# Sewer56/dxt-lossless-transform

Hardware: AMD Instinct MI355X
Metric: GiB/s BC blocks transformed (fwd+inv) (higher is better)
Workload: dtype u8

## Files before the change

dxt-lossless-transform_amd/csrc/batch_api.cpp:

```cpp
#include <hip/hip_runtime_api.h>

#include <algorithm>
#include <cstring>
#include <vector>

#include "../../include/dxtlt_gfx950.h"
#include "batch_tables.h"
#include "bcn_launch.h"
#include "granule_launch.h"
#include "host_common.h"

namespace {

using namespace dxtlt_host;
using dxtlt::BatchEntry;

const char* const kDeviceFormatText = "batch item: format must be 1..5 (BC1..BC5), 6 (BC6H) or 7 (BC7; 6 and 7 are this build's own formats; "
                                      "pixel formats 8 and 9 go through dxtlt_transform_batch_host or the calls of dxtlt_pixels.h)";
const char* const kHostFormatText = "batch item: format must be 1..5 (BC1..BC5), 6 (BC6H), 7 (BC7), 8 (4-byte pixels) or 9 (3-byte pixels; "
                                    "6 to 9 are this build's own formats)";

inline bool pixel_item_overlaps(const DxtltBatchItem& it)
{
    if (!is_pixel_format(it.format) || it.len == 0)
        return false;
    const uintptr_t a = reinterpret_cast<uintptr_t>(it.d_input), b = reinterpret_cast<uintptr_t>(it.d_output);
    return a < b + it.len && b < a + it.len;
}

int32_t launch_pixel_item(const DxtltBatchItem& it, void* stream)
{
    const uint64_t pixels = it.len / item_block_bytes(it.format);
    return pixel_device_range(pixel_bytes_of(it.format), it.inverse != 0, it.d_input, it.d_output, pixels, 0, pixels,
                              pixel_decorrelate_of(it.decorrelation_mode),
                              pixel_layout_of(it.split_alpha_endpoints != 0, it.split_colour_endpoints != 0), stream);
}

thread_local dxtlt_host::TableRing g_ring;

const bool kTableByCopyEngine = dxtlt::experiment_env("DXTLT_BATCH_TABLE_COPY") != nullptr && dxtlt::experiment_env("DXTLT_BATCH_TABLE_COPY")[0] == '1';

}

dxtlt_host::TableRing& dxtlt_host::thread_table_ring() { return g_ring; }

hipError_t dxtlt_host::upload_table(TableSlot* slot, size_t bytes, hipStream_t stream)
{
    if (kTableByCopyEngine)
        return hipMemcpyAsync(slot->dev, slot->host, bytes, hipMemcpyHostToDevice, stream);
    return dxtlt::launch_table_upload(slot->host_mapped, slot->dev, bytes, stream);
}

void dxtlt_host::release_batch_thread_tables() { g_ring.release(); }

int32_t dxtlt_host::batch_item_defect(const DxtltBatchItem& it, int max_format, bool host_call)
{
    if (it.format < 1 || it.format > max_format)
        return fail(kInvalidArgument, host_call ? kHostFormatText : kDeviceFormatText);
    if (it.len % item_block_bytes(it.format) != 0)
        return fail(kInvalidLength, "batch item: len is not a multiple of the block size");
    if (it.decorrelation_mode > 3 && dxtlt::format_has_colour(it.format))
        return fail(kInvalidArgument, "batch item: decorrelation_mode must be 0..3");
    if (it.len > 0 && (it.d_input == nullptr || it.d_output == nullptr))
        return fail(kInvalidArgument, host_call ? "batch item: NULL buffer with len > 0" : "batch item: NULL device buffer with len > 0");
    if (pixel_item_overlaps(it))
        return fail(kInvalidArgument, "batch item: pixel input and output overlap");
    if (host_call && it.len >= (size_t(4) << 30))
        return fail(kInvalidArgument, "batch item of 4 GiB or more: use the single-buffer entry point");
    return kOk;
}

namespace {

inline dxtlt::Settings item_settings(const DxtltBatchItem& it)
{
    dxtlt::Settings s{};
    s.variant = it.decorrelation_mode;
    s.split_alpha = it.split_alpha_endpoints != 0;
    s.split_colour = it.split_colour_endpoints != 0;
    return dxtlt::effective_settings((dxtlt::Format)it.format, s);
}

struct TileLaunch {
    int key = 0;
    std::vector<BatchEntry> entries;
    uint32_t wgs = 0;
    uint32_t uniform_wgs = 0;
    bool strided = false;
    int64_t src_stride = 0, dst_stride = 0;
    bool wide = false;
    size_t at = 0, entry_bytes = 0;

    dxtlt::Format format() const { return (dxtlt::Format)((key >> 5) + 1); }
    bool inverse() const { return ((key >> 4) & 1) != 0; }
};

using GranuleEntry = dxtlt::granule::BatchEntry;
struct GranuleLaunch {
    std::vector<GranuleEntry> entries, tails;
    std::vector<uint32_t> coarse;
    uint64_t wgs = 0;
    size_t items = 0;
    size_t at = 0, entry_bytes = 0, tail_bytes = 0, bytes = 0;
};

struct BatchPlan {
    GranuleLaunch granules[4];
    std::vector<TileLaunch> tiles;
    std::vector<size_t> singles;
    std::vector<size_t> pixels;
    size_t table_bytes = 0;
};
inline int granule_format(int q) { return q < 2 ? 7 : 6; }

int32_t plan_batch(const DxtltBatchItem* items, size_t count, bool pixels_allowed, BatchPlan& plan)
{
    if (count == 0)
        return kOk;
    if (items == nullptr)
        return fail(kInvalidArgument, "NULL item array with count > 0");
    for (size_t i = 0; i < count; ++i)
        if (int32_t rc = batch_item_defect(items[i], pixels_allowed ? 9 : 7, false); rc != kOk)
            return rc;
    for (const int format : {7, 6}) {
        uint64_t granules[2] = {0, 0};
        for (size_t i = 0; i < count; ++i)
            if (items[i].format == format)
                granules[items[i].inverse ? 1 : 0] += items[i].len / 16 / 1024;
        if (granules[0] > 0xFFFFFFull || granules[1] > 0xFFFFFFull)
            return fail(kInvalidArgument, dxtlt::granule::named(format, "batch too large for one launch (256 GiB or more of ", " in one direction)"));
    }

    int launch_of_key[5 * 2 * 16];
    for (int& l : launch_of_key)
        l = -1;
    for (size_t i = 0; i < count; ++i) {
        const DxtltBatchItem& it = items[i];
        if (it.len == 0 || dxtlt::granule::is_granule_format(it.format))
            continue;
        if (is_pixel_format(it.format)) {
            plan.pixels.push_back(i);
            continue;
        }
        if (it.len >= (size_t(64) << 30))
            return fail(kInvalidArgument, "batch item of 64 GiB or more: use the single-buffer entry point");
        const dxtlt::Settings s = item_settings(it);
        const int key = (((it.format - 1) * 2 + (it.inverse ? 1 : 0)) << 4) | settings_code(s);
        int li = launch_of_key[key];
        BatchEntry e{};
        e.src = static_cast<const uint8_t*>(it.d_input);
        e.dst = static_cast<uint8_t*>(it.d_output);
        e.blocks = it.len / item_block_bytes(it.format);
        e.first_wg = li >= 0 ? plan.tiles[(size_t)li].wgs : 0;
        const uint32_t wgs = dxtlt::plan_batch_entry((dxtlt::Format)it.format, it.inverse != 0, s, e);
        if (wgs == 0xFFFFFFFFu) {
            plan.singles.push_back(i);
            continue;
        }
        if (li < 0) {
            li = launch_of_key[key] = (int)plan.tiles.size();
            plan.tiles.emplace_back();
            plan.tiles.back().key = key;
            plan.tiles.back().uniform_wgs = wgs;
        }
        TileLaunch& l = plan.tiles[(size_t)li];
        if ((uint64_t)l.wgs + wgs > 0xFFFFFFull)
            return fail(kInvalidArgument, "batch too large for one launch (64 GiB or more of one format, direction and settings)");
        l.wgs += wgs;
        l.entries.push_back(e);
        if (wgs != l.uniform_wgs)
            l.uniform_wgs = 0;
    }
    std::sort(plan.tiles.begin(), plan.tiles.end(), [](const TileLaunch& a, const TileLaunch& b) { return a.key < b.key; });
    static const bool no_uniform = dxtlt::experiment_env("DXTLT_BATCH_NO_UNIFORM") != nullptr;
    static const bool no_strided = dxtlt::experiment_env("DXTLT_BATCH_NO_STRIDED") != nullptr;
    for (TileLaunch& l : plan.tiles) {
        const size_t n = l.entries.size();
        if (no_uniform)
            l.uniform_wgs = 0;
        l.strided = l.uniform_wgs != 0 && !no_strided;
        l.src_stride = n >= 2 ? (int64_t)(l.entries[1].src - l.entries[0].src) : 0;
        l.dst_stride = n >= 2 ? (int64_t)(l.entries[1].dst - l.entries[0].dst) : 0;
        for (size_t i = 1; i < n && l.strided; ++i) {
            const BatchEntry &a = l.entries[0], &b = l.entries[i];
            l.strided = b.blocks == a.blocks && b.full_tiles == a.full_tiles && b.form == a.form && b.halo_vecs == a.halo_vecs &&
                        std::memcmp(b.shift, a.shift, sizeof a.shift) == 0 && std::memcmp(b.gbase, a.gbase, sizeof a.gbase) == 0 &&
                        b.src == a.src + (int64_t)i * l.src_stride && b.dst == a.dst + (int64_t)i * l.dst_stride;
        }
    }

    for (int q = 0; q < 4; ++q) {
        GranuleLaunch& p = plan.granules[q];
        const int inverse = q & 1, format = granule_format(q);
        for (size_t i = 0; i < count; ++i) {
            const DxtltBatchItem& it = items[i];
            if (it.format != format || it.len == 0 || (it.inverse != 0) != (inverse != 0))
                continue;
            const uint64_t blocks = it.len / 16, tail = blocks % 1024, main = blocks - tail;
            const uint8_t* src = static_cast<const uint8_t*>(it.d_input);
            uint8_t* dst = static_cast<uint8_t*>(it.d_output);
            ++p.items;
            if (main != 0) {
                p.entries.push_back({src, dst, main, (uint32_t)p.wgs, 0});
                p.wgs += main / 1024;
            }
            if (tail != 0)
                p.tails.push_back({src + main * 16, dst + main * 16, 0, 0, (uint32_t)tail});
        }
        if (p.items == 0)
            continue;
        p.coarse.resize(coarse_index_count((uint32_t)p.wgs));
        build_coarse_index(p.entries.data(), p.entries.size(), (uint32_t)p.wgs, p.coarse.data());
        p.entry_bytes = p.entries.size() * sizeof(GranuleEntry);
        p.tail_bytes = p.tails.size() * sizeof(GranuleEntry);
        p.bytes = padded(p.entry_bytes + p.tail_bytes + p.coarse.size() * sizeof(uint32_t), 16);
        p.at = plan.table_bytes;
        plan.table_bytes += p.bytes;
    }
    for (TileLaunch& l : plan.tiles) {
        l.entry_bytes = padded(l.entries.size() * sizeof(BatchEntry), 16);
        l.at = plan.table_bytes;
        plan.table_bytes += l.entry_bytes + dxtlt::batch_index_bytes(l.wgs);
    }
    return kOk;
}

void fill_tables(BatchPlan& plan, uint8_t* host)
{
    for (const GranuleLaunch& p : plan.granules) {
        uint8_t* h = host + p.at;
        if (p.entry_bytes) std::memcpy(h, p.entries.data(), p.entry_bytes);
        if (p.tail_bytes) std::memcpy(h + p.entry_bytes, p.tails.data(), p.tail_bytes);
        if (!p.coarse.empty()) std::memcpy(h + p.entry_bytes + p.tail_bytes, p.coarse.data(), p.coarse.size() * sizeof(uint32_t));
    }
    for (TileLaunch& l : plan.tiles) {
        std::memcpy(host + l.at, l.entries.data(), l.entries.size() * sizeof(BatchEntry));
        l.wide = dxtlt::build_batch_index(l.entries.data(), l.entries.size(), l.wgs, host + l.at + l.entry_bytes);
    }
}

}

int32_t dxtlt_host::batch_device(const DxtltBatchItem* items, size_t count, void* hip_stream, bool pixels_allowed)
{
    BatchPlan plan;
    if (int32_t rc = plan_batch(items, count, pixels_allowed, plan); rc != kOk)
        return rc;
    hipStream_t user = static_cast<hipStream_t>(hip_stream);
    if (plan.table_bytes != 0) {
        StagedTables tables;
        hipError_t e = tables.acquire(plan.table_bytes);
        if (e != hipSuccess)
            return fail(kDevice, "batch table staging", e);
        fill_tables(plan, tables.host());
        e = tables.upload(user);
        const char* what = "batch table copy / launch";
        for (int q = 0; q < 4 && e == hipSuccess; ++q) {
            const GranuleLaunch& p = plan.granules[q];
            if (p.bytes == 0)
                continue;
            const uint8_t* d = tables.dev() + p.at;
            e = dxtlt::granule::launch_batch(granule_format(q), (q & 1) != 0, reinterpret_cast<const GranuleEntry*>(d),
                                             reinterpret_cast<const uint32_t*>(d + p.entry_bytes + p.tail_bytes), (uint32_t)p.entries.size(),
                                             (uint32_t)p.wgs, reinterpret_cast<const GranuleEntry*>(d + p.entry_bytes),
                                             (uint32_t)p.tails.size(), user);
            if (e != hipSuccess)
                what = granule_format(q) == 7 ? "BC7 batch table copy / launch" : "BC6H batch table copy / launch";
        }
        for (size_t k = 0; k < plan.tiles.size() && e == hipSuccess; ++k) {
            const TileLaunch& l = plan.tiles[k];
            const uint8_t* d = tables.dev() + l.at;
            e = dxtlt::launch_batch(l.format(), l.inverse(), settings_of_code(l.key & 15), reinterpret_cast<const BatchEntry*>(d),
                                    d + l.entry_bytes, (uint32_t)l.entries.size(), l.wgs, l.uniform_wgs, l.wide, user,
                                    l.strided ? &l.entries[0] : nullptr, l.src_stride, l.dst_stride);
        }
        if (int32_t rc = tables.finish(e, user, what, "batch event"); rc != kOk)
            return rc;
    }
    for (size_t i : plan.singles) {
        const DxtltBatchItem& it = items[i];
        const uint64_t blocks = it.len / item_block_bytes(it.format);
        HIP_TRY(dxtlt::launch_transform((dxtlt::Format)it.format, it.inverse != 0, item_settings(it), it.d_input, it.d_output,
                                        dxtlt::Range{blocks, 0, blocks}, user),
                "batch item launch");
    }
    for (size_t i : plan.pixels)
        if (int32_t rc = launch_pixel_item(items[i], user); rc != kOk)
            return rc;
    return kOk;
}

namespace {

void* address(uint64_t a) { return reinterpret_cast<void*>(static_cast<uintptr_t>(a)); }

}

extern "C" int32_t dxtlt_transform_batch_device(const DxtltBatchItem* items, size_t count, void* hip_stream)
{
    return batch_device(items, count, hip_stream, false);
}

extern "C" uint32_t dxtlt_debug_plan_batch(int32_t format, int32_t inverse, int32_t variant, int32_t split_alpha, int32_t split_colour,
                                           const uint64_t* src_addresses, const uint64_t* dst_addresses, const uint64_t* blocks, size_t count,
                                           DxtltDebugPlannedEntry* entries_out, uint8_t* index_out, size_t index_capacity,
                                           uint32_t* index_is_wide_out)
{
    if (index_is_wide_out)
        *index_is_wide_out = 0;
    if (format < 1 || format > 5 || (count != 0 && (!src_addresses || !dst_addresses || !blocks || !entries_out)))
// ... 2 lines not shown
    for (size_t i = 0; i < count; ++i) {
        if (blocks[i] >= (uint64_t(64) << 30) / item_block_bytes((uint8_t)format))
            return 0xFFFFFFFFu;
        items[i] = DxtltBatchItem{address(src_addresses[i]), address(dst_addresses[i]), blocks[i] * item_block_bytes((uint8_t)format),
                                  (uint8_t)format, (uint8_t)(inverse != 0), (uint8_t)std::min<uint32_t>((uint32_t)variant, 255),
                                  (uint8_t)(split_alpha != 0), (uint8_t)(split_colour != 0), {0, 0, 0}};
    }
    BatchPlan plan;
    if (plan_batch(items.data(), count, false, plan) != kOk || !plan.singles.empty())
        return 0xFFFFFFFFu;
    static const TileLaunch none;
    const TileLaunch& l = plan.tiles.empty() ? none : plan.tiles[0];
    if (l.wgs != 0 && (index_out == nullptr || index_capacity < dxtlt::batch_index_bytes(l.wgs)))
        return 0xFFFFFFFFu;
    size_t k = 0;
    for (size_t i = 0; i < count; ++i) {
        DxtltDebugPlannedEntry& o = entries_out[i];
        o = DxtltDebugPlannedEntry{};
        if (blocks[i] == 0) {
            o.first_wg = o.end_wg = k < l.entries.size() ? l.entries[k].first_wg : l.wgs;
            continue;
        }
        const BatchEntry& e = l.entries[k++];
        o.first_wg = e.first_wg;
        o.end_wg = e.end_wg;
        o.full_tiles = e.full_tiles;
        o.form = e.form;
        o.halo_vecs = e.halo_vecs;
        std::memcpy(o.shift, e.shift, sizeof o.shift);
        std::memcpy(o.gbase, e.gbase, sizeof o.gbase);
    }
    if (l.wgs != 0) {
        std::vector<uint8_t> tables(plan.table_bytes);
        fill_tables(plan, tables.data());
        std::memcpy(index_out, tables.data() + plan.tiles[0].at + plan.tiles[0].entry_bytes, dxtlt::batch_index_bytes(l.wgs));
        if (index_is_wide_out)
            *index_is_wide_out = plan.tiles[0].wide ? 1 : 0;
    }
    return l.wgs;
}

extern "C" int32_t dxtlt_debug_plan_batch_call(const DxtltBatchItem* items, size_t count, int32_t pixels_allowed, DxtltDebugBatchLaunch* out,
                                               size_t cap, uint64_t* table_bytes_out)
{
    if (table_bytes_out)
        *table_bytes_out = 0;
    BatchPlan plan;
    if (plan_batch(items, count, pixels_allowed != 0, plan) != kOk)
        return -1;
    std::vector<uint8_t> tables(plan.table_bytes);
    fill_tables(plan, tables.data());
    if (table_bytes_out)
        *table_bytes_out = plan.table_bytes;
    size_t n = 0;
    auto put = [&](const DxtltDebugBatchLaunch& r) {
        if (out != nullptr && n < cap)
            out[n] = r;
        ++n;
    };
    for (int q = 0; q < 4; ++q) {
        const GranuleLaunch& p = plan.granules[q];
        if (p.bytes == 0)
            continue;
        DxtltDebugBatchLaunch r{};
        r.kind = 0, r.format = granule_format(q), r.inverse = q & 1;
        r.items = (uint32_t)p.items, r.entries = (uint32_t)p.entries.size(), r.tails = (uint32_t)p.tails.size(), r.workgroups = (uint32_t)p.wgs;
        r.table_offset = p.at, r.table_bytes = p.bytes;
        put(r);
    }
    for (const TileLaunch& l : plan.tiles) {
        DxtltDebugBatchLaunch r{};
        r.kind = 1, r.format = l.format(), r.inverse = l.inverse() ? 1 : 0, r.settings_code = l.key & 15;
        r.items = r.entries = (uint32_t)l.entries.size(), r.workgroups = l.wgs;
        r.uniform_wgs = l.uniform_wgs, r.strided = l.strided ? 1 : 0, r.wide = l.wide ? 1 : 0;
        r.src_stride = l.src_stride, r.dst_stride = l.dst_stride;
        r.table_offset = l.at, r.table_bytes = l.entry_bytes + dxtlt::batch_index_bytes(l.wgs);
        put(r);
    }
    for (int kind = 2; kind <= 3; ++kind)
        for (size_t i : kind == 2 ? plan.singles : plan.pixels) {
            DxtltDebugBatchLaunch r{};
            r.kind = kind, r.format = items[i].format, r.inverse = items[i].inverse ? 1 : 0;
            r.settings_code = kind == 2 ? settings_code(item_settings(items[i])) : 0;
            r.items = r.entries = 1, r.first_item = i;
            put(r);
        }
    return (int32_t)n;
}

extern "C" int32_t dxtlt_debug_plan_batch_granules(const DxtltBatchItem* items, size_t count, int32_t format, int32_t inverse,
                                                   uint32_t* first_wg_out, uint64_t* main_blocks_out, size_t entry_cap, uint32_t* coarse_out,
                                                   size_t coarse_cap)
{
    BatchPlan plan;
    if (!dxtlt::granule::is_granule_format(format) || plan_batch(items, count, false, plan) != kOk)
        return -1;
    std::vector<uint8_t> tables(plan.table_bytes);
    fill_tables(plan, tables.data());
    const GranuleLaunch& p = plan.granules[(format == 7 ? 0 : 2) + (inverse != 0 ? 1 : 0)];
    if (p.bytes == 0)
        return 0;
    const GranuleEntry* entries = reinterpret_cast<const GranuleEntry*>(tables.data() + p.at);
    const uint32_t* coarse = reinterpret_cast<const uint32_t*>(tables.data() + p.at + p.entry_bytes + p.tail_bytes);
    for (size_t k = 0; k < p.entries.size() && k < entry_cap; ++k) {
        if (first_wg_out) first_wg_out[k] = entries[k].first_wg;
        if (main_blocks_out) main_blocks_out[k] = entries[k].main_blocks;
    }
    for (size_t k = 0; k < p.coarse.size() && k < coarse_cap && coarse_out != nullptr; ++k)
        coarse_out[k] = coarse[k];
    return (int32_t)p.coarse.size();
}
```

dxt-lossless-transform_amd/csrc/batch_kernels.hip:

```cpp
#include <cstdlib>
#include <cstring>
#include <vector>

#include "bcn_device.h"

#include "batch_lookup.h"

namespace dxtlt {

struct BatchView {
    const uint8_t* src;
    uint8_t* dst;
    uint64_t blocks;
    uint32_t first_wg, end_wg, full_tiles;
    uint32_t flags;
    uint32_t shifts[2];
    uint64_t gbase[6];
};

__device__ __forceinline__ BatchView load_batch_entry(const BatchEntry* entry)
{
    const uint64_t* q = reinterpret_cast<const uint64_t*>(entry);
    const uint32_t* w = reinterpret_cast<const uint32_t*>(entry);
    BatchView v;
// ... 128 lines not shown
    for (int i = 0; i < 6; ++i) {
        sh.d[i] = (int)((en.shifts[i >> 2] >> (8 * (i & 3))) & 127u);
        sh.gbase[i] = en.gbase[i];
    }
#ifdef DXTLT_EXPERIMENTS
    sh.xcd_remap = 0;
    sh.line_policy = INVERSE ? 1 : 3;
    sh.skip_partial = 0;
#endif
    sh.natural = 1;
    sh.halo_vecs = (int)(en.flags >> 8) & 0xFF;
    sh.full_tiles = en.full_tiles;
    sh.range_blocks = en.blocks;
    if constexpr (INVERSE) {
        if (local < en.full_tiles) {
            const uint64_t tile = xcd_contiguous_tile(local, en.full_tiles);
            inv_shift_tile<FMT, VARIANT, SA, SC, THREADS>(en.src, en.dst, en.blocks, 0, sh, tile, lds);
            WG_TIMING_END(2);
            return;
        }
        inv_shift_edge_tile<FMT, VARIANT, SA, SC, THREADS>(en.src, en.dst, en.blocks, sh, en.full_tiles, lds);
        WG_TIMING_END(4);
    } else {
        if (local != 0 && local < en.full_tiles) {
            fwd_halo_tile<FMT, VARIANT, SA, SC, kNormNone, true, THREADS>(en.src, en.dst, en.blocks, 0, sh, local, lds);
            WG_TIMING_END(2);
            return;
        }
        fwd_halo_edge_tile<FMT, VARIANT, SA, SC, kNormNone, true, THREADS>(en.src, en.dst, sh, local, lds);
        WG_TIMING_END(local == 0 ? 3 : 4);
    }
}

uint32_t plan_batch_entry(Format fmt, bool inverse, const Settings& s, BatchEntry& e)
{
    if (e.blocks == 0)
        return 0;
    const Settings es = effective_settings(fmt, s);
    const Streams S = make_streams(fmt, es.split_alpha, es.split_colour);
    const void* soa = inverse ? (const void*)e.src : (const void*)e.dst;
    const uint64_t T = (uint64_t)tile_blocks(fmt, batch_tile_threads(fmt, es.split_colour, inverse));
    const uint64_t tiles = e.blocks / T, rest = e.blocks % T;
    const uint64_t mask = inverse ? 15 : (uint64_t)(kHaloAlign - 1);
    bool on_lines = true, stream_tails = false;
    int d[6] = {0, 0, 0, 0, 0, 0}, halo_blocks = 0;
    for (int i = 0; i < S.n; ++i) {
        const uint64_t base = reinterpret_cast<uintptr_t>(soa) + (uint64_t)S.off[i] * e.blocks;
        d[i] = (int)(base & mask);
        on_lines = on_lines && (base & 127) == 0;
        stream_tails = stream_tails || d[i] != 0;
        halo_blocks = std::max(halo_blocks, (d[i] + S.width[i] - 1) / S.width[i]);
    }
    if (!shifts_are_natural(S, d))
        return 0xFFFFFFFFu;
    e.form = on_lines ? 1 : 0;
    e.natural = 1;
    e.reserved = 0;
    e.reserved2[0] = e.reserved2[1] = 0;
    const int per_vec = 16 / fmt_block(fmt);
    e.halo_vecs = inverse ? 0 : (uint8_t)((halo_blocks + per_vec - 1) / per_vec);
    for (int i = 0; i < 6; ++i) {
        e.shift[i] = (uint8_t)d[i];
        e.gbase[i] = i < S.n ? (uint64_t)S.off[i] * e.blocks - (uint64_t)d[i] : 0;
    }
    e.full_tiles = (uint32_t)tiles;
    const bool edge = rest != 0 || (!inverse && stream_tails);
    const uint32_t wgs = (uint32_t)tiles + (edge ? 1u : 0u);
    e.end_wg = e.first_wg + wgs;
    return wgs;
}

namespace {

using BatchFn = void (*)(const BatchEntry*, const uint8_t*, uint32_t, uint32_t, uint32_t, StridedBatch);

template <int FMT, int VARIANT, bool SA, bool SC>
BatchFn batch_fn(bool inverse) { return inverse ? batch_kernel<FMT, VARIANT, SA, SC, true> : batch_kernel<FMT, VARIANT, SA, SC, false>; }

template <int FMT, int VARIANT>
BatchFn batch_splits(bool sa, bool sc, bool inverse)
{
    if constexpr (FMT == kBc3) {
        if (sa)
            return sc ? batch_fn<FMT, VARIANT, true, true>(inverse) : batch_fn<FMT, VARIANT, true, false>(inverse);
    }
    return sc ? batch_fn<FMT, VARIANT, false, true>(inverse) : batch_fn<FMT, VARIANT, false, false>(inverse);
}

template <int FMT>
BatchFn batch_bc45(bool split_endpoints, bool inverse)
{
    return split_endpoints ? batch_fn<FMT, kNone, true, false>(inverse) : batch_fn<FMT, kNone, false, false>(inverse);
}

template <int FMT>
BatchFn batch_variant(int variant, bool sa, bool sc, bool inverse)
{
    switch (variant) {
    case kNone: return batch_splits<FMT, kNone>(sa, sc, inverse);
    case kVar1: return batch_splits<FMT, kVar1>(sa, sc, inverse);
    case kVar2: return batch_splits<FMT, kVar2>(sa, sc, inverse);
    default: return batch_splits<FMT, kVar3>(sa, sc, inverse);
// ... 48 lines not shown
```

dxt-lossless-transform_amd/csrc/bcn_launch.h:

```cpp
#pragma once
#include <hip/hip_runtime_api.h>
#include <stddef.h>
#include <stdint.h>

#include <algorithm>
#include <cstdlib>
#include <cstring>
#include <vector>

namespace dxtlt {

inline const char* experiment_env(const char* name)
{
#ifdef DXTLT_EXPERIMENTS
    return std::getenv(name);
#else
    (void)name;
    return nullptr;
#endif
}

enum Format : int { kBc1 = 1, kBc2 = 2, kBc3 = 3, kBc4 = 4, kBc5 = 5 };

struct Settings {
    int variant;
    bool split_alpha;
    bool split_colour;
    int normalize = 0;
};

struct Range {
    uint64_t total_blocks;
    uint64_t first_block;
    uint64_t num_blocks;
};

struct LaunchTuning {
    int tile_threads;
    int force_generic;
// ... 41 lines not shown
hipError_t launch_normalize_bc23_blocks(int fmt, const void* in, void* out, uint64_t num_blocks, int alpha_mode, int color_mode,
                                        hipStream_t stream);
hipError_t launch_normalize_bc23_all_modes(int fmt, const void* in, void* const* outs, uint64_t num_blocks, hipStream_t stream);
hipError_t launch_normalize_bc2_split(void* colours, void* indices, uint64_t num_blocks, int color_mode, hipStream_t stream);
hipError_t launch_normalize_bc3_split(void* alpha_endpoints, void* alpha_indices, void* color_endpoints, void* color_indices,
                                      uint64_t num_blocks, int alpha_mode, int color_mode, hipStream_t stream);

struct BatchEntry {
    const uint8_t* src;
    uint8_t* dst;
    uint64_t blocks;
    uint32_t first_wg;
    uint32_t end_wg;
    uint32_t full_tiles;
    uint8_t form;
    uint8_t halo_vecs;
    uint8_t natural;
    uint8_t reserved;
    uint8_t shift[6];
    uint8_t reserved2[2];
    uint64_t gbase[6];
};
static_assert(sizeof(BatchEntry) == 96, "BatchEntry layout is shared between host and device");

constexpr uint32_t kBatchIndexWgs = 64, kBatchBaseWgs = 4096;
inline size_t batch_index_base_count(uint32_t total_wgs) { return ((size_t)total_wgs + kBatchBaseWgs - 1) / kBatchBaseWgs; }
inline size_t batch_index_delta_count(uint32_t total_wgs) { return ((size_t)total_wgs + kBatchIndexWgs - 1) / kBatchIndexWgs; }
inline size_t batch_index_bytes(uint32_t total_wgs)
{
    return (batch_index_base_count(total_wgs) * 4 + 2 * batch_index_delta_count(total_wgs) + 15) & ~(size_t)15;
}

uint32_t plan_batch_entry(Format fmt, bool inverse, const Settings& s, BatchEntry& e);

hipError_t launch_table_upload(const void* host_mapped, void* dev, size_t bytes, hipStream_t stream);

hipError_t launch_batch(Format fmt, bool inverse, const Settings& s, const BatchEntry* d_entries, const uint8_t* d_index,
                        uint32_t n_entries, uint32_t total_wgs, uint32_t uniform_wgs, bool wide_index, hipStream_t stream,
                        const BatchEntry* strided_first = nullptr, int64_t src_stride = 0, int64_t dst_stride = 0);

inline bool build_batch_index(const BatchEntry* entries, size_t n_entries, uint32_t total_wgs, uint8_t* index)
{
    const size_t n_base = batch_index_base_count(total_wgs), n_delta = batch_index_delta_count(total_wgs);
    uint32_t* base = reinterpret_cast<uint32_t*>(index);
    std::memset(index, 0, batch_index_bytes(total_wgs));
    std::vector<uint32_t> d(n_delta);
    uint32_t largest = 0;
    size_t cur = 0;
    for (size_t j = 0; j < n_delta; ++j) {
        const uint32_t wg = (uint32_t)(j * kBatchIndexWgs);
        while (cur + 1 < n_entries && entries[cur].end_wg <= wg)
            ++cur;
        if (wg % kBatchBaseWgs == 0)
            base[wg / kBatchBaseWgs] = (uint32_t)cur;
        d[j] = (uint32_t)(cur - base[wg / kBatchBaseWgs]);
        largest = std::max(largest, d[j]);
    }
    const bool wide = largest > 255;
    uint8_t* delta = index + n_base * 4;
    for (size_t j = 0; j < n_delta; ++j) {
        if (wide) {
            delta[2 * j] = (uint8_t)d[j];
            delta[2 * j + 1] = (uint8_t)(d[j] >> 8);
        } else {
            delta[j] = (uint8_t)d[j];
        }
    }
    return wide;
}

hipError_t launch_tiled_array(Format fmt, bool inverse, const Settings& s, const void* first_src, void* first_dst,
                              uint64_t blocks, uint32_t n_buffers, int64_t src_stride, int64_t dst_stride, hipStream_t stream);

inline int block_bytes(Format f) { return f == kBc1 || f == kBc4 ? 8 : 16; }

constexpr bool format_has_alpha_split(int fmt) { return fmt == kBc3 || fmt == kBc4 || fmt == kBc5; }
constexpr bool format_has_colour(int fmt) { return fmt == kBc1 || fmt == kBc2 || fmt == kBc3; }
inline Settings effective_settings(Format f, const Settings& s)
{
    Settings e = s;
    e.split_alpha = format_has_alpha_split(f) && s.split_alpha;
    if (!format_has_colour(f)) {
        e.variant = 0;
        e.split_colour = false;
    }
    return e;
}

struct Streams {
    int n;
    int width[6];
    int off[6];
};

constexpr Streams make_streams(int fmt, bool split_alpha, bool split_colour)
{
    Streams s{};
    int n = 0, off = 0;
    if (fmt == kBc4 || fmt == kBc5) {
        for (int h = 0; h < (fmt == kBc5 ? 2 : 1); ++h) {
            if (split_alpha) {
                s.width[n] = 1; s.off[n] = off; off += 1; ++n;
                s.width[n] = 1; s.off[n] = off; off += 1; ++n;
// ... 33 lines not shown
```

include/dxtlt_gfx950.h:

```cpp
#ifndef DXTLT_GFX950_H
#define DXTLT_GFX950_H

#include <stdbool.h>
#include <stddef.h>
#include <stdint.h>

#include "dlt_size_estimator.h"

#ifdef __cplusplus
extern "C" {
#endif

#define DXTLT_OK 0
#define DXTLT_E_INVALID_LENGTH 1
#define DXTLT_E_INVALID_ARGUMENT 2
#define DXTLT_E_NO_DEVICE 3
#define DXTLT_E_DEVICE 4
#define DXTLT_E_ESTIMATOR 5
#define DXTLT_E_ALLOCATION 6

#define DXTLT_YCOCG_NONE 0
#define DXTLT_YCOCG_VARIANT1 1
#define DXTLT_YCOCG_VARIANT2 2
#define DXTLT_YCOCG_VARIANT3 3
// ... 67 lines not shown
} DxtltBatchItem;
int32_t dxtlt_transform_batch_device(const DxtltBatchItem *items, size_t count, void *hip_stream);
typedef struct DxtltDebugPlannedEntry {
    uint32_t first_wg, end_wg;
    uint32_t full_tiles;
    uint8_t form;
    uint8_t halo_vecs;
    uint8_t shift[6];
    uint64_t gbase[6];
} DxtltDebugPlannedEntry;
uint32_t dxtlt_debug_plan_batch(int32_t format, int32_t inverse, int32_t variant, int32_t split_alpha, int32_t split_colour,
                                const uint64_t *src_addresses, const uint64_t *dst_addresses, const uint64_t *blocks, size_t count,
                                DxtltDebugPlannedEntry *entries_out, uint8_t *index_out, size_t index_capacity,
                                uint32_t *index_is_wide_out);
typedef struct DxtltDebugBatchLaunch {
    int32_t kind;
    int32_t format;
    int32_t inverse;
    int32_t settings_code;
    uint32_t items;
    uint32_t entries;
    uint32_t tails;
    uint32_t workgroups;
    uint32_t uniform_wgs;
    uint32_t strided;
    uint32_t wide;
    int64_t src_stride, dst_stride;
    uint64_t table_offset;
    uint64_t table_bytes;
    uint64_t first_item;
} DxtltDebugBatchLaunch;
int32_t dxtlt_debug_plan_batch_call(const DxtltBatchItem *items, size_t count, int32_t pixels_allowed, DxtltDebugBatchLaunch *out,
                                    size_t cap, uint64_t *table_bytes_out);
int32_t dxtlt_debug_plan_batch_granules(const DxtltBatchItem *items, size_t count, int32_t format, int32_t inverse,
                                        uint32_t *first_wg_out, uint64_t *main_blocks_out, size_t entry_cap, uint32_t *coarse_out,
                                        size_t coarse_cap);
int32_t dxtlt_debug_plan_batch_host(const uint64_t *len, size_t count, uint64_t chunk_cap_bytes, uint32_t *chunk_of_item_out,
                                    uint64_t *slot_out, uint64_t *chunk_bytes_out, size_t chunk_cap, uint64_t *arena_bytes_out);

typedef struct DxtltDebugPlannedLaunch {
    int32_t kind;
    int32_t threads;
    uint32_t workgroups;
    uint32_t full_tiles;
    uint64_t range_blocks;
    uint64_t aos_offset;
    uint8_t shift[6];
    uint8_t halo_vecs;
    uint8_t natural;
    uint64_t gbase[6];
} DxtltDebugPlannedLaunch;
int32_t dxtlt_debug_plan_transform(int32_t format, int32_t inverse, int32_t variant, int32_t split_alpha, int32_t split_colour,
                                   uint64_t src_address, uint64_t dst_address, uint64_t total_blocks, uint64_t first_block,
                                   uint64_t num_blocks, DxtltDebugPlannedLaunch *out, int32_t cap);

int32_t dxtlt_transform_batch_host(const DxtltBatchItem *items, size_t count);

int32_t dxtlt_transform_sharded(int32_t format, bool inverse, const uint8_t *input_ptr, uint8_t *output_ptr,
                                size_t len, uint8_t decorrelation_mode, bool split_alpha_endpoints,
                                bool split_colour_endpoints, int32_t num_devices);

typedef struct DxtltShardStat {
    int32_t device;
    int32_t cpus_bound;
    uint64_t first_block;
    uint64_t blocks;
// ... 25 lines not shown
```

Measured before the change: 3197.

## Cut host batch planning overhead and skip table upload for strided launches

```diff
diff --git a/dxt-lossless-transform_amd/csrc/batch_api.cpp b/dxt-lossless-transform_amd/csrc/batch_api.cpp
--- a/dxt-lossless-transform_amd/csrc/batch_api.cpp
+++ b/dxt-lossless-transform_amd/csrc/batch_api.cpp
@@ -1,6 +1,7 @@
 #include <hip/hip_runtime_api.h>
 
 #include <algorithm>
+#include <chrono>
 #include <cstring>
 #include <vector>
 
@@ -57,7 +58,8 @@
 {
     if (it.format < 1 || it.format > max_format)
         return fail(kInvalidArgument, host_call ? kHostFormatText : kDeviceFormatText);
-    if (it.len % item_block_bytes(it.format) != 0)
+    const uint32_t block = item_block_bytes(it.format);
+    if ((block & (block - 1)) == 0 ? (it.len & (block - 1)) != 0 : it.len % block != 0)
         return fail(kInvalidLength, "batch item: len is not a multiple of the block size");
     if (it.decorrelation_mode > 3 && dxtlt::format_has_colour(it.format))
         return fail(kInvalidArgument, "batch item: decorrelation_mode must be 0..3");
@@ -86,13 +88,25 @@
     std::vector<BatchEntry> entries;
     uint32_t wgs = 0;
     uint32_t uniform_wgs = 0;
+    bool regular = true;
     bool strided = false;
     int64_t src_stride = 0, dst_stride = 0;
     bool wide = false;
     size_t at = 0, entry_bytes = 0;
+    size_t staged_at = 0;
 
     dxtlt::Format format() const { return (dxtlt::Format)((key >> 5) + 1); }
     bool inverse() const { return ((key >> 4) & 1) != 0; }
+    void restart(int new_key)
+    {
+        key = new_key;
+        entries.clear();
+        wgs = uniform_wgs = 0;
+        regular = true;
+        strided = wide = false;
+        src_stride = dst_stride = 0;
+        at = entry_bytes = staged_at = 0;
+    }
 };
 
 using GranuleEntry = dxtlt::granule::BatchEntry;
@@ -102,103 +116,85 @@
     uint64_t wgs = 0;
     size_t items = 0;
     size_t at = 0, entry_bytes = 0, tail_bytes = 0, bytes = 0;
+
+    void restart()
+    {
+        entries.clear(), tails.clear(), coarse.clear();
+        wgs = 0;
+        items = at = entry_bytes = tail_bytes = bytes = 0;
+    }
 };
 
 struct BatchPlan {
     GranuleLaunch granules[4];
     std::vector<TileLaunch> tiles;
+    std::vector<TileLaunch> spare;
     std::vector<size_t> singles;
     std::vector<size_t> pixels;
+    dxtlt::BatchEntryPlanner planner_of_key[5 * 2 * 16];
+    bool planner_ready[5 * 2 * 16] = {};
     size_t table_bytes = 0;
+    size_t staged_bytes = 0;
+
+    void restart()
+    {
+        for (GranuleLaunch& p : granules)
+            p.restart();
+        for (TileLaunch& l : tiles)
+            spare.push_back(std::move(l));
+        tiles.clear(), singles.clear(), pixels.clear();
+        table_bytes = staged_bytes = 0;
+    }
+    TileLaunch& open(int key, size_t count)
+    {
+        size_t pick = spare.size();
+        if (tiles.empty())
+            for (size_t k = 0; k < spare.size(); ++k)
+                if (pick == spare.size() || spare[k].entries.capacity() > spare[pick].entries.capacity())
+                    pick = k;
+        if (pick < spare.size())
+            std::swap(spare[pick], spare.back());
+        if (spare.empty()) {
+            tiles.emplace_back();
+        } else {
+            tiles.push_back(std::move(spare.back()));
+            spare.pop_back();
+        }
+        TileLaunch& l = tiles.back();
+        l.restart(key);
+        if (tiles.size() == 1)
+            l.entries.reserve(std::min(count, size_t(1) << 20));
+        return l;
+    }
 };
 inline int granule_format(int q) { return q < 2 ? 7 : 6; }
 
 int32_t plan_batch(const DxtltBatchItem* items, size_t count, bool pixels_allowed, BatchPlan& plan)
 {
+    plan.restart();
     if (count == 0)
         return kOk;
     if (items == nullptr)
         return fail(kInvalidArgument, "NULL item array with count > 0");
-    for (size_t i = 0; i < count; ++i)
-        if (int32_t rc = batch_item_defect(items[i], pixels_allowed ? 9 : 7, false); rc != kOk)
-            return rc;
-    for (const int format : {7, 6}) {
-        uint64_t granules[2] = {0, 0};
-        for (size_t i = 0; i < count; ++i)
-            if (items[i].format == format)
-                granules[items[i].inverse ? 1 : 0] += items[i].len / 16 / 1024;
-        if (granules[0] > 0xFFFFFFull || granules[1] > 0xFFFFFFull)
-            return fail(kInvalidArgument, dxtlt::granule::named(format, "batch too large for one launch (256 GiB or more of ", " in one direction)"));
-    }
-
+    const int max_format = pixels_allowed ? 9 : 7;
+    const char* too_large = nullptr;
+    uint64_t granule_total[4] = {0, 0, 0, 0};
     int launch_of_key[5 * 2 * 16];
     for (int& l : launch_of_key)
         l = -1;
     for (size_t i = 0; i < count; ++i) {
         const DxtltBatchItem& it = items[i];
-        if (it.len == 0 || dxtlt::granule::is_granule_format(it.format))
-            continue;
-        if (is_pixel_format(it.format)) {
-            plan.pixels.push_back(i);
-            continue;
-        }
-        if (it.len >= (size_t(64) << 30))
-            return fail(kInvalidArgument, "batch item of 64 GiB or more: use the single-buffer entry point");
-        const dxtlt::Settings s = item_settings(it);
-        const int key = (((it.format - 1) * 2 + (it.inverse ? 1 : 0)) << 4) | settings_code(s);
-        int li = launch_of_key[key];
-        BatchEntry e{};
-        e.src = static_cast<const uint8_t*>(it.d_input);
-        e.dst = static_cast<uint8_t*>(it.d_output);
-        e.blocks = it.len / item_block_bytes(it.format);
-        e.first_wg = li >= 0 ? plan.tiles[(size_t)li].wgs : 0;
-        const uint32_t wgs = dxtlt::plan_batch_entry((dxtlt::Format)it.format, it.inverse != 0, s, e);
-        if (wgs == 0xFFFFFFFFu) {
-            plan.singles.push_back(i);
-            continue;
-        }
-        if (li < 0) {
-            li = launch_of_key[key] = (int)plan.tiles.size();
-            plan.tiles.emplace_back();
-            plan.tiles.back().key = key;
-            plan.tiles.back().uniform_wgs = wgs;
-        }
-        TileLaunch& l = plan.tiles[(size_t)li];
-        if ((uint64_t)l.wgs + wgs > 0xFFFFFFull)
-            return fail(kInvalidArgument, "batch too large for one launch (64 GiB or more of one format, direction and settings)");
-        l.wgs += wgs;
-        l.entries.push_back(e);
-        if (wgs != l.uniform_wgs)
-            l.uniform_wgs = 0;
-    }
-    std::sort(plan.tiles.begin(), plan.tiles.end(), [](const TileLaunch& a, const TileLaunch& b) { return a.key < b.key; });
-    static const bool no_uniform = dxtlt::experiment_env("DXTLT_BATCH_NO_UNIFORM") != nullptr;
-    static const bool no_strided = dxtlt::experiment_env("DXTLT_BATCH_NO_STRIDED") != nullptr;
-    for (TileLaunch& l : plan.tiles) {
-        const size_t n = l.entries.size();
-        if (no_uniform)
-            l.uniform_wgs = 0;
-        l.strided = l.uniform_wgs != 0 && !no_strided;
-        l.src_stride = n >= 2 ? (int64_t)(l.entries[1].src - l.entries[0].src) : 0;
-        l.dst_stride = n >= 2 ? (int64_t)(l.entries[1].dst - l.entries[0].dst) : 0;
-        for (size_t i = 1; i < n && l.strided; ++i) {
-            const BatchEntry &a = l.entries[0], &b = l.entries[i];
-            l.strided = b.blocks == a.blocks && b.full_tiles == a.full_tiles && b.form == a.form && b.halo_vecs == a.halo_vecs &&
-                        std::memcmp(b.shift, a.shift, sizeof a.shift) == 0 && std::memcmp(b.gbase, a.gbase, sizeof a.gbase) == 0 &&
-                        b.src == a.src + (int64_t)i * l.src_stride && b.dst == a.dst + (int64_t)i * l.dst_stride;
-        }
-    }
-
-    for (int q = 0; q < 4; ++q) {
-        GranuleLaunch& p = plan.granules[q];
-        const int inverse = q & 1, format = granule_format(q);
-        for (size_t i = 0; i < count; ++i) {
-            const DxtltBatchItem& it = items[i];
-            if (it.format != format || it.len == 0 || (it.inverse != 0) != (inverse != 0))
-                continue;
+        if (int32_t rc = batch_item_defect(it, max_format, false); rc != kOk)
+            return rc;
+        if (it.len == 0)
+            continue;
+        if (dxtlt::granule::is_granule_format(it.format)) {
+            const int q = (it.format == 7 ? 0 : 2) + (it.inverse ? 1 : 0);
+            GranuleLaunch& p = plan.granules[q];
             const uint64_t blocks = it.len / 16, tail = blocks % 1024, main = blocks - tail;
             const uint8_t* src = static_cast<const uint8_t*>(it.d_input);
             uint8_t* dst = static_cast<uint8_t*>(it.d_output);
+            granule_total[q] += main / 1024;
             ++p.items;
             if (main != 0) {
                 p.entries.push_back({src, dst, main, (uint32_t)p.wgs, 0});
@@ -206,7 +202,89 @@
             }
             if (tail != 0)
                 p.tails.push_back({src + main * 16, dst + main * 16, 0, 0, (uint32_t)tail});
-        }
+            continue;
+        }
+        if (is_pixel_format(it.format)) {
+            plan.pixels.push_back(i);
+            continue;
+        }
+        if (too_large != nullptr)
+            continue;
+        if (it.len >= (size_t(64) << 30)) {
+            too_large = "batch item of 64 GiB or more: use the single-buffer entry point";
+            continue;
+        }
+        const dxtlt::Settings s = item_settings(it);
+        const int key = (((it.format - 1) * 2 + (it.inverse ? 1 : 0)) << 4) | settings_code(s);
+        if (!plan.planner_ready[key]) {
+            plan.planner_of_key[key] = dxtlt::make_batch_entry_planner((dxtlt::Format)it.format, it.inverse != 0, s);
+            plan.planner_ready[key] = true;
+        }
+        int li = launch_of_key[key];
+        const bool opened = li < 0;
+        if (opened) {
+            li = launch_of_key[key] = (int)plan.tiles.size();
+            plan.open(key, count);
+        }
+        TileLaunch& l = plan.tiles[(size_t)li];
+        const size_t n = l.entries.size();
+        l.entries.emplace_back();
+        BatchEntry& e = l.entries[n];
+        e.src = static_cast<const uint8_t*>(it.d_input);
+        e.dst = static_cast<uint8_t*>(it.d_output);
+        e.blocks = it.len >> (it.format == 1 || it.format == 4 ? 3 : 4);
+        e.first_wg = l.wgs;
+        const uint32_t wgs = dxtlt::plan_batch_entry(plan.planner_of_key[key], e);
+        bool taken = wgs != 0xFFFFFFFFu;
+        if (!taken) {
+            plan.singles.push_back(i);
+        } else if ((uint64_t)l.wgs + wgs > 0xFFFFFFull) {
+            too_large = "batch too large for one launch (64 GiB or more of one format, direction and settings)";
+            taken = false;
+        }
+        if (!taken) {
+            l.entries.pop_back();
+            if (opened) {
+                plan.spare.push_back(std::move(plan.tiles.back()));
+                plan.tiles.pop_back();
+                launch_of_key[key] = -1;
+            }
+            continue;
+        }
+        l.wgs += wgs;
+        if (opened)
+            l.uniform_wgs = wgs;
+        else if (wgs != l.uniform_wgs)
+            l.uniform_wgs = 0;
+        if (n == 1) {
+            l.src_stride = (int64_t)(reinterpret_cast<uintptr_t>(e.src) - reinterpret_cast<uintptr_t>(l.entries[0].src));
+            l.dst_stride = (int64_t)(reinterpret_cast<uintptr_t>(e.dst) - reinterpret_cast<uintptr_t>(l.entries[0].dst));
+        }
+        if (n >= 1 && l.regular) {
+            const BatchEntry& a = l.entries[0];
+            l.regular = e.blocks == a.blocks && ((dxtlt::batch_entry_form_word(e) ^ dxtlt::batch_entry_form_word(a)) & 0xFFFFu) == 0 &&
+                        dxtlt::batch_entry_shift_word(e) == dxtlt::batch_entry_shift_word(a) &&
+                        reinterpret_cast<uintptr_t>(e.src) == reinterpret_cast<uintptr_t>(a.src) + (uint64_t)n * (uint64_t)l.src_stride &&
+                        reinterpret_cast<uintptr_t>(e.dst) == reinterpret_cast<uintptr_t>(a.dst) + (uint64_t)n * (uint64_t)l.dst_stride;
+        }
+    }
+    for (const int q : {0, 2})
+        if (granule_total[q] > 0xFFFFFFull || granule_total[q + 1] > 0xFFFFFFull)
+            return fail(kInvalidArgument, dxtlt::granule::named(granule_format(q), "batch too large for one launch (256 GiB or more of ", " in one direction)"));
+    if (too_large != nullptr)
+        return fail(kInvalidArgument, too_large);
+
+    if (plan.tiles.size() > 1)
+        std::sort(plan.tiles.begin(), plan.tiles.end(), [](const TileLaunch& a, const TileLaunch& b) { return a.key < b.key; });
+    static const bool no_uniform = dxtlt::experiment_env("DXTLT_BATCH_NO_UNIFORM") != nullptr;
+    static const bool no_strided = dxtlt::experiment_env("DXTLT_BATCH_NO_STRIDED") != nullptr;
+    for (TileLaunch& l : plan.tiles) {
+        if (no_uniform)
+            l.uniform_wgs = 0;
+        l.strided = l.uniform_wgs != 0 && !no_strided && l.regular;
+    }
+
+    for (GranuleLaunch& p : plan.granules) {
         if (p.items == 0)
             continue;
         p.coarse.resize(coarse_index_count((uint32_t)p.wgs));
@@ -217,15 +295,21 @@
         p.at = plan.table_bytes;
         plan.table_bytes += p.bytes;
     }
+    plan.staged_bytes = plan.table_bytes;
     for (TileLaunch& l : plan.tiles) {
         l.entry_bytes = padded(l.entries.size() * sizeof(BatchEntry), 16);
+        const size_t bytes = l.entry_bytes + dxtlt::batch_index_bytes(l.wgs);
         l.at = plan.table_bytes;
-        plan.table_bytes += l.entry_bytes + dxtlt::batch_index_bytes(l.wgs);
+        plan.table_bytes += bytes;
+        if (!l.strided) {
+            l.staged_at = plan.staged_bytes;
+            plan.staged_bytes += bytes;
+        }
     }
     return kOk;
 }
 
-void fill_tables(BatchPlan& plan, uint8_t* host)
+void fill_tables(BatchPlan& plan, uint8_t* host, bool staged)
 {
     for (const GranuleLaunch& p : plan.granules) {
         uint8_t* h = host + p.at;
@@ -234,48 +318,79 @@
         if (!p.coarse.empty()) std::memcpy(h + p.entry_bytes + p.tail_bytes, p.coarse.data(), p.coarse.size() * sizeof(uint32_t));
     }
     for (TileLaunch& l : plan.tiles) {
-        std::memcpy(host + l.at, l.entries.data(), l.entries.size() * sizeof(BatchEntry));
-        l.wide = dxtlt::build_batch_index(l.entries.data(), l.entries.size(), l.wgs, host + l.at + l.entry_bytes);
-    }
+        if (staged && l.strided)
+            continue;
+        uint8_t* h = host + (staged ? l.staged_at : l.at);
+        std::memcpy(h, l.entries.data(), l.entries.size() * sizeof(BatchEntry));
+        l.wide = dxtlt::build_batch_index(l.entries.data(), l.entries.size(), l.wgs, h + l.entry_bytes);
+    }
+}
+
+struct CallReport {
+    uint64_t calls = 0, items_walked = 0, bytes_staged = 0, host_ns = 0;
+    uint32_t upload_launched = 0;
+    bool time_host = false;
+};
+thread_local CallReport t_report;
+thread_local BatchPlan t_plan;
+
+inline uint64_t host_clock_ns(bool on)
+{
+    return on ? (uint64_t)std::chrono::duration_cast<std::chrono::nanoseconds>(std::chrono::steady_clock::now().time_since_epoch()).count() : 0;
+}
+void report_call(const BatchPlan& plan, size_t count, uint64_t began_ns)
+{
+    ++t_report.calls;
+    t_report.items_walked = count;
+    t_report.bytes_staged = plan.staged_bytes;
+    t_report.upload_launched = plan.staged_bytes != 0 ? 1 : 0;
+    t_report.host_ns = t_report.time_host ? host_clock_ns(true) - began_ns : 0;
 }
 
 }
 
 int32_t dxtlt_host::batch_device(const DxtltBatchItem* items, size_t count, void* hip_stream, bool pixels_allowed)
 {
-    BatchPlan plan;
+    const uint64_t began_ns = host_clock_ns(t_report.time_host);
+    BatchPlan& plan = t_plan;
     if (int32_t rc = plan_batch(items, count, pixels_allowed, plan); rc != kOk)
         return rc;
     hipStream_t user = static_cast<hipStream_t>(hip_stream);
-    if (plan.table_bytes != 0) {
-        StagedTables tables;
-        hipError_t e = tables.acquire(plan.table_bytes);
+    StagedTables tables;
+    const bool staged = plan.staged_bytes != 0;
+    if (staged) {
+        if (hipError_t e = tables.acquire(plan.staged_bytes); e != hipSuccess)
+            return fail(kDevice, "batch table staging", e);
+        fill_tables(plan, tables.host(), true);
+    }
+    report_call(plan, count, began_ns);
+    hipError_t e = staged ? tables.upload(user) : hipSuccess;
+    const uint8_t* dev = staged ? tables.dev() : nullptr;
+    const char* what = "batch table copy / launch";
+    for (int q = 0; q < 4 && e == hipSuccess; ++q) {
+        const GranuleLaunch& p = plan.granules[q];
+        if (p.bytes == 0)
+            continue;
+        const uint8_t* d = dev + p.at;
+        e = dxtlt::granule::launch_batch(granule_format(q), (q & 1) != 0, reinterpret_cast<const GranuleEntry*>(d),
+                                         reinterpret_cast<const uint32_t*>(d + p.entry_bytes + p.tail_bytes), (uint32_t)p.entries.size(),
+                                         (uint32_t)p.wgs, reinterpret_cast<const GranuleEntry*>(d + p.entry_bytes),
+                                         (uint32_t)p.tails.size(), user);
         if (e != hipSuccess)
-            return fail(kDevice, "batch table staging", e);
-        fill_tables(plan, tables.host());
-        e = tables.upload(user);
-        const char* what = "batch table copy / launch";
-        for (int q = 0; q < 4 && e == hipSuccess; ++q) {
-            const GranuleLaunch& p = plan.granules[q];
-            if (p.bytes == 0)
-                continue;
-            const uint8_t* d = tables.dev() + p.at;
-            e = dxtlt::granule::launch_batch(granule_format(q), (q & 1) != 0, reinterpret_cast<const GranuleEntry*>(d),
-                                             reinterpret_cast<const uint32_t*>(d + p.entry_bytes + p.tail_bytes), (uint32_t)p.entries.size(),
-                                             (uint32_t)p.wgs, reinterpret_cast<const GranuleEntry*>(d + p.entry_bytes),
-                                             (uint32_t)p.tails.size(), user);
-            if (e != hipSuccess)
-                what = granule_format(q) == 7 ? "BC7 batch table copy / launch" : "BC6H batch table copy / launch";
-        }
-        for (size_t k = 0; k < plan.tiles.size() && e == hipSuccess; ++k) {
-            const TileLaunch& l = plan.tiles[k];
-            const uint8_t* d = tables.dev() + l.at;
-            e = dxtlt::launch_batch(l.format(), l.inverse(), settings_of_code(l.key & 15), reinterpret_cast<const BatchEntry*>(d),
-                                    d + l.entry_bytes, (uint32_t)l.entries.size(), l.wgs, l.uniform_wgs, l.wide, user,
-                                    l.strided ? &l.entries[0] : nullptr, l.src_stride, l.dst_stride);
-        }
+            what = granule_format(q) == 7 ? "BC7 batch table copy / launch" : "BC6H batch table copy / launch";
+    }
+    for (size_t k = 0; k < plan.tiles.size() && e == hipSuccess; ++k) {
+        const TileLaunch& l = plan.tiles[k];
+        const uint8_t* d = l.strided ? nullptr : dev + l.staged_at;
+        e = dxtlt::launch_batch(l.format(), l.inverse(), settings_of_code(l.key & 15), reinterpret_cast<const BatchEntry*>(d),
+                                l.strided ? nullptr : d + l.entry_bytes, (uint32_t)l.entries.size(), l.wgs, l.uniform_wgs, l.wide, user,
+                                l.strided ? &l.entries[0] : nullptr, l.src_stride, l.dst_stride);
+    }
+    if (staged) {
         if (int32_t rc = tables.finish(e, user, what, "batch event"); rc != kOk)
             return rc;
+    } else if (e != hipSuccess) {
+        return fail(kDevice, what, e);
     }
     for (size_t i : plan.singles) {
         const DxtltBatchItem& it = items[i];
@@ -344,7 +459,7 @@
     }
     if (l.wgs != 0) {
         std::vector<uint8_t> tables(plan.table_bytes);
-        fill_tables(plan, tables.data());
+        fill_tables(plan, tables.data(), false);
         std::memcpy(index_out, tables.data() + plan.tiles[0].at + plan.tiles[0].entry_bytes, dxtlt::batch_index_bytes(l.wgs));
         if (index_is_wide_out)
             *index_is_wide_out = plan.tiles[0].wide ? 1 : 0;
@@ -357,11 +472,17 @@
 {
     if (table_bytes_out)
         *table_bytes_out = 0;
-    BatchPlan plan;
+    const uint64_t began_ns = host_clock_ns(t_report.time_host);
+    BatchPlan& plan = t_plan;
     if (plan_batch(items, count, pixels_allowed != 0, plan) != kOk)
         return -1;
+    static thread_local std::vector<uint8_t> slot;
+    if (slot.size() < plan.staged_bytes)
+        slot.resize(plan.staged_bytes);
+    fill_tables(plan, slot.data(), true);
+    report_call(plan, count, began_ns);
     std::vector<uint8_t> tables(plan.table_bytes);
-    fill_tables(plan, tables.data());
+    fill_tables(plan, tables.data(), false);
     if (table_bytes_out)
         *table_bytes_out = plan.table_bytes;
     size_t n = 0;
@@ -408,7 +529,7 @@
     if (!dxtlt::granule::is_granule_format(format) || plan_batch(items, count, false, plan) != kOk)
         return -1;
     std::vector<uint8_t> tables(plan.table_bytes);
-    fill_tables(plan, tables.data());
+    fill_tables(plan, tables.data(), false);
     const GranuleLaunch& p = plan.granules[(format == 7 ? 0 : 2) + (inverse != 0 ? 1 : 0)];
     if (p.bytes == 0)
         return 0;
@@ -422,3 +543,17 @@
         coarse_out[k] = coarse[k];
     return (int32_t)p.coarse.size();
 }
+
+extern "C" void dxtlt_debug_batch_last_call(DxtltDebugBatchCallReport* out)
+{
+    if (out == nullptr)
+        return;
+    out->calls = t_report.calls;
+    out->items_walked = t_report.items_walked;
+    out->bytes_staged = t_report.bytes_staged;
+    out->host_ns = t_report.host_ns;
+    out->upload_launched = t_report.upload_launched;
+    out->reserved = 0;
+}
+
+extern "C" void dxtlt_debug_batch_time_host(int32_t on) { t_report.time_host = on != 0; }
diff --git a/dxt-lossless-transform_amd/csrc/batch_kernels.hip b/dxt-lossless-transform_amd/csrc/batch_kernels.hip
--- a/dxt-lossless-transform_amd/csrc/batch_kernels.hip
+++ b/dxt-lossless-transform_amd/csrc/batch_kernels.hip
@@ -184,42 +184,31 @@
     }
 }
 
-uint32_t plan_batch_entry(Format fmt, bool inverse, const Settings& s, BatchEntry& e)
-{
-    if (e.blocks == 0)
-        return 0;
+BatchEntryPlanner make_batch_entry_planner(Format fmt, bool inverse, const Settings& s)
+{
     const Settings es = effective_settings(fmt, s);
     const Streams S = make_streams(fmt, es.split_alpha, es.split_colour);
-    const void* soa = inverse ? (const void*)e.src : (const void*)e.dst;
-    const uint64_t T = (uint64_t)tile_blocks(fmt, batch_tile_threads(fmt, es.split_colour, inverse));
-    const uint64_t tiles = e.blocks / T, rest = e.blocks % T;
-    const uint64_t mask = inverse ? 15 : (uint64_t)(kHaloAlign - 1);
-    bool on_lines = true, stream_tails = false;
-    int d[6] = {0, 0, 0, 0, 0, 0}, halo_blocks = 0;
+    BatchEntryPlanner P;
+    P.n = S.n;
     for (int i = 0; i < S.n; ++i) {
-        const uint64_t base = reinterpret_cast<uintptr_t>(soa) + (uint64_t)S.off[i] * e.blocks;
-        d[i] = (int)(base & mask);
-        on_lines = on_lines && (base & 127) == 0;
-        stream_tails = stream_tails || d[i] != 0;
-        halo_blocks = std::max(halo_blocks, (d[i] + S.width[i] - 1) / S.width[i]);
-    }
-    if (!shifts_are_natural(S, d))
-        return 0xFFFFFFFFu;
-    e.form = on_lines ? 1 : 0;
-    e.natural = 1;
-    e.reserved = 0;
-    e.reserved2[0] = e.reserved2[1] = 0;
-    const int per_vec = 16 / fmt_block(fmt);
-    e.halo_vecs = inverse ? 0 : (uint8_t)((halo_blocks + per_vec - 1) / per_vec);
-    for (int i = 0; i < 6; ++i) {
-        e.shift[i] = (uint8_t)d[i];
-        e.gbase[i] = i < S.n ? (uint64_t)S.off[i] * e.blocks - (uint64_t)d[i] : 0;
-    }
-    e.full_tiles = (uint32_t)tiles;
-    const bool edge = rest != 0 || (!inverse && stream_tails);
-    const uint32_t wgs = (uint32_t)tiles + (edge ? 1u : 0u);
-    e.end_wg = e.first_wg + wgs;
-    return wgs;
+        P.off[i] = (uint32_t)S.off[i];
+        P.width[i] = (uint32_t)S.width[i];
+        P.recip[i] = (65536u + (uint32_t)S.width[i] - 1) / (uint32_t)S.width[i];
+        P.element_mask[i] = (uint32_t)stream_element_width(S.width[i]) - 1;
+    }
+    P.tile_blocks = (uint64_t)tile_blocks(fmt, batch_tile_threads(fmt, es.split_colour, inverse));
+    if ((P.tile_blocks & (P.tile_blocks - 1)) == 0)
+        for (P.tile_shift = 0; (uint64_t(1) << P.tile_shift) != P.tile_blocks;)
+            ++P.tile_shift;
+    P.shift_mask = inverse ? 15 : (uint64_t)(kHaloAlign - 1);
+    P.per_vec_shift = fmt_block(fmt) == 8 ? 1 : 0;
+    P.inverse = inverse;
+    return P;
+}
+
+uint32_t plan_batch_entry(Format fmt, bool inverse, const Settings& s, BatchEntry& e)
+{
+    return plan_batch_entry(make_batch_entry_planner(fmt, inverse, s), e);
 }
 
 namespace {
diff --git a/dxt-lossless-transform_amd/csrc/bcn_launch.h b/dxt-lossless-transform_amd/csrc/bcn_launch.h
--- a/dxt-lossless-transform_amd/csrc/bcn_launch.h
+++ b/dxt-lossless-transform_amd/csrc/bcn_launch.h
@@ -5,6 +5,7 @@
 
 #include <algorithm>
 #include <cstdlib>
+#include <cstddef>
 #include <cstring>
 #include <vector>
 
@@ -112,6 +113,19 @@
 }
 
 uint32_t plan_batch_entry(Format fmt, bool inverse, const Settings& s, BatchEntry& e);
+struct BatchEntryPlanner {
+    int n = 0;
+    uint32_t off[6] = {};
+    uint32_t width[6] = {};
+    uint32_t recip[6] = {};
+    uint32_t element_mask[6] = {};
+    uint64_t tile_blocks = 0;
+    int tile_shift = -1;
+    uint64_t shift_mask = 0;
+    uint32_t per_vec_shift = 0;
+    bool inverse = false;
+};
+BatchEntryPlanner make_batch_entry_planner(Format fmt, bool inverse, const Settings& s);
 
 hipError_t launch_table_upload(const void* host_mapped, void* dev, size_t bytes, hipStream_t stream);
 
@@ -149,6 +163,56 @@
     return wide;
 }
 
+static_assert(offsetof(BatchEntry, form) == 36 && offsetof(BatchEntry, halo_vecs) == 37 && offsetof(BatchEntry, natural) == 38 &&
+                  offsetof(BatchEntry, shift) == 40 && offsetof(BatchEntry, gbase) == 48,
+              "plan_batch_entry writes BatchEntry's byte fields as words");
+inline uint32_t batch_entry_form_word(const BatchEntry& e)
+{
+    uint32_t w;
+    std::memcpy(&w, reinterpret_cast<const uint8_t*>(&e) + 36, 4);
+    return w;
+}
+inline uint64_t batch_entry_shift_word(const BatchEntry& e)
+{
+    uint64_t w;
+    std::memcpy(&w, reinterpret_cast<const uint8_t*>(&e) + 40, 8);
+    return w;
+}
+inline uint32_t plan_batch_entry(const BatchEntryPlanner& P, BatchEntry& e)
+{
+    if (e.blocks == 0)
+        return 0;
+    const uint64_t soa = reinterpret_cast<uintptr_t>(P.inverse ? (const void*)e.src : (const void*)e.dst);
+    const uint64_t tiles = P.tile_shift >= 0 ? e.blocks >> P.tile_shift : e.blocks / P.tile_blocks;
+    const uint64_t rest = e.blocks - tiles * P.tile_blocks;
+    uint64_t off_lines = 0, shifts = 0;
+    uint32_t unnatural = 0, halo_blocks = 0;
+    for (int i = 0; i < 6; ++i) {
+        if (i >= P.n) {
+            e.gbase[i] = 0;
+            continue;
+        }
+        const uint64_t base = soa + (uint64_t)P.off[i] * e.blocks;
+        const uint32_t d = (uint32_t)(base & P.shift_mask);
+        off_lines |= base & 127;
+        shifts |= (uint64_t)d << (8 * i);
+        unnatural |= d & P.element_mask[i];
+        halo_blocks = std::max(halo_blocks, ((d + P.width[i] - 1) * P.recip[i]) >> 16);
+        e.gbase[i] = (uint64_t)P.off[i] * e.blocks - (uint64_t)d;
+    }
+    if (unnatural != 0)
+        return 0xFFFFFFFFu;
+    const uint32_t halo_vecs = P.inverse ? 0 : ((halo_blocks + (1u << P.per_vec_shift) - 1) >> P.per_vec_shift) & 0xFFu;
+    const uint32_t form_word = (off_lines == 0 ? 1u : 0u) | (halo_vecs << 8) | (1u << 16);
+    std::memcpy(reinterpret_cast<uint8_t*>(&e) + 36, &form_word, 4);
+    std::memcpy(reinterpret_cast<uint8_t*>(&e) + 40, &shifts, 8);
+    e.full_tiles = (uint32_t)tiles;
+    const bool edge = rest != 0 || (!P.inverse && shifts != 0);
+    const uint32_t wgs = (uint32_t)tiles + (edge ? 1u : 0u);
+    e.end_wg = e.first_wg + wgs;
+    return wgs;
+}
+
 hipError_t launch_tiled_array(Format fmt, bool inverse, const Settings& s, const void* first_src, void* first_dst,
                               uint64_t blocks, uint32_t n_buffers, int64_t src_stride, int64_t dst_stride, hipStream_t stream);
 
diff --git a/include/dxtlt_gfx950.h b/include/dxtlt_gfx950.h
--- a/include/dxtlt_gfx950.h
+++ b/include/dxtlt_gfx950.h
@@ -123,6 +123,16 @@
 } DxtltDebugBatchLaunch;
 int32_t dxtlt_debug_plan_batch_call(const DxtltBatchItem *items, size_t count, int32_t pixels_allowed, DxtltDebugBatchLaunch *out,
                                     size_t cap, uint64_t *table_bytes_out);
+typedef struct DxtltDebugBatchCallReport {
+    uint64_t calls;
+    uint64_t items_walked;
+    uint64_t bytes_staged;
+    uint64_t host_ns;
+    uint32_t upload_launched;
+    uint32_t reserved;
+} DxtltDebugBatchCallReport;
+void dxtlt_debug_batch_last_call(DxtltDebugBatchCallReport *out);
+void dxtlt_debug_batch_time_host(int32_t on);
 int32_t dxtlt_debug_plan_batch_granules(const DxtltBatchItem *items, size_t count, int32_t format, int32_t inverse,
                                         uint32_t *first_wg_out, uint64_t *main_blocks_out, size_t entry_cap, uint32_t *coarse_out,
                                         size_t coarse_cap);
```

Result: slower. 3165 (-1.0%).
